# sihan-shao/QuantizationAwareTHzDOE

Measured on AMD Instinct MI355X. Metric: complex-field propagations/sec (N×N) + achieved HBM GB/s at 1/2/4/8 GPU, higher is better.
Workload: dtype complex64 (fp32)

## Files before the change

include/thzdoe.h:

```cpp
#ifndef THZDOE_H_
#define THZDOE_H_

#include <stddef.h>

#ifdef __cplusplus
extern "C" {
#endif

#define THZ_OK 0
#define THZ_E_ARG 1
#define THZ_E_UNSUPPORTED 2
#define THZ_E_WORKSPACE 3
#define THZ_E_HIP 4

#define THZ_BANDLIMIT_NONE 0
#define THZ_BANDLIMIT_EXACT 1
#define THZ_BANDLIMIT_APPROX 2

#define THZ_MAX_WAVELENGTHS 64
#define THZ_MAX_Z 256

typedef void* thz_stream_t;

#define THZ_ABI_VERSION 9

const char* thz_version(void);
const char* thz_last_error(void);
int thz_abi_version(void);

typedef struct thz_asm_desc {
  int B, C, H, W;
  int pad_h, pad_w;
  int unpad;
  int bandlimit;
  int Z;
  int adjoint;
  int z_chunk;
  float dx, dy;
  const float* wavelengths;
  const float* z;
  const struct thz_aperture_desc* window_mask;
  const float* z_dev;
} thz_asm_desc;

int thz_asm_workspace_size(const thz_asm_desc* d, size_t* bytes);
int thz_asm_forward(const thz_asm_desc* d, const void* in, void* out, void* workspace, size_t workspace_bytes,
                    thz_stream_t stream);
int thz_asm_slice_workspace_size(const thz_asm_desc* d, size_t* bytes);
int thz_asm_slice_forward(const thz_asm_desc* d, int row, const void* in, void* out ,
                          void* workspace, size_t workspace_bytes, thz_stream_t stream);
int thz_asm_slice_adjoint_workspace_size(const thz_asm_desc* d, size_t* bytes);
int thz_asm_slice_adjoint(const thz_asm_desc* d, int row, const void* grad_out ,
                          void* grad_in , void* workspace, size_t workspace_bytes,
                          thz_stream_t stream);
int thz_asm_band(const thz_asm_desc* d, int* ncols, int* z_chunk);
int thz_asm_transfer_function(const thz_asm_desc* d, void* out, thz_stream_t stream);

typedef struct thz_czt_desc {
  int B, C, H, W;
  int outH, outW;
  float dx, dy;
  float odx, ody;
  float z;
  const float* wavelengths;
  int adjoint;
} thz_czt_desc;

int thz_czt_workspace_size(const thz_czt_desc* d, size_t* bytes);
int thz_czt_forward(const thz_czt_desc* d, const void* in, void* out, void* workspace, size_t workspace_bytes,
                    thz_stream_t stream);

typedef struct thz_czt_slice_desc {
  int B, C, H, W;
  int outH, outW;
  float dx, dy, odx, ody;
  int Z;
  const float* z;
  const float* wavelengths;
  int row;
} thz_czt_slice_desc;

int thz_czt_slice_workspace_size(const thz_czt_slice_desc* d, size_t* bytes);
int thz_czt_slice_forward(const thz_czt_slice_desc* d, const void* in ,
                          void* out , void* workspace, size_t workspace_bytes,
                          thz_stream_t stream);
int thz_czt_slice_adjoint_workspace_size(const thz_czt_slice_desc* d, size_t* bytes);
int thz_czt_slice_adjoint(const thz_czt_slice_desc* d, const void* grad_out ,
                          void* grad_in , void* workspace, size_t workspace_bytes,
                          thz_stream_t stream);

typedef struct thz_rsc_desc {
  int B, C, H, W;
  int vectorial;
  float dx, dy;
  float z;
  const float* wavelengths;
  int adjoint;
} thz_rsc_desc;

int thz_rsc_workspace_size(const thz_rsc_desc* d, size_t* bytes);
int thz_rsc_forward(const thz_rsc_desc* d, const void* in, void* out, void* workspace, size_t workspace_bytes,
                    thz_stream_t stream);

typedef struct thz_rsc_slice_desc {
  int B, C, H, W;
  int vectorial;
  float dx, dy;
  int Z;
// ... 202 lines not shown
```

quantizationawarethzdoe_amd/_lib.py:

```python
from __future__ import annotations

import ctypes
import os
import threading

_HERE = os.path.dirname(os.path.abspath(__file__))
LIB_PATH = os.environ.get("THZDOE_LIB", os.path.join(_HERE, "libthzdoe.so"))

THZ_OK = 0
THZ_E_ARG = 1
THZ_E_UNSUPPORTED = 2
THZ_E_WORKSPACE = 3
THZ_E_HIP = 4
THZ_MAX_WAVELENGTHS = 64
THZ_MAX_Z = 256
THZ_ABI_VERSION = 9

BANDLIMIT = {None: 0, False: 0, "none": 0, "exact": 1, "approx": 2}

EXPORTED = [
    "thz_version", "thz_last_error", "thz_abi_version",
    "thz_asm_workspace_size", "thz_asm_forward", "thz_asm_band", "thz_asm_forward_modulated",
    "thz_asm_forward_loss", "thz_asm_adjoint_loss", "thz_asm_transfer_function", "thz_rs_kernel",
    "thz_asm_slice_workspace_size", "thz_asm_slice_forward",
    "thz_asm_slice_adjoint_workspace_size", "thz_asm_slice_adjoint",
    "thz_czt_workspace_size", "thz_czt_forward",
    "thz_czt_slice_workspace_size", "thz_czt_slice_forward",
    "thz_czt_slice_adjoint_workspace_size", "thz_czt_slice_adjoint",
    "thz_rsc_workspace_size", "thz_rsc_forward",
    "thz_rsc_slice_workspace_size", "thz_rsc_slice_forward",
    "thz_rsc_slice_adjoint_workspace_size", "thz_rsc_slice_adjoint",
    "thz_doe_modulate_forward", "thz_doe_modulate_backward", "thz_quant_forward", "thz_quant_backward",
    "thz_doe_quant_backward", "thz_radial_quant_backward",
    "thz_radial_forward", "thz_radial_backward",
    "thz_gaussian_beam", "thz_thin_lens", "thz_aperture",
    "thz_intensity_mse_workspace_size", "thz_intensity_mse_forward", "thz_intensity_mse_backward",
    "thz_resample_forward", "thz_resample_backward",
    "thz_fft_rows",
    "thz_asm64_workspace_size", "thz_asm64_forward", "thz_czt64_workspace_size", "thz_czt64_forward",
    "thz_rsc64_workspace_size", "thz_rsc64_forward", "thz_fft64_rows",
    "thz_step_fetch", "thz_adam_step",
    "thz_timing_enable", "thz_timing_reset", "thz_timing_read",
]


class ThzError(RuntimeError):

    def __init__(self, code, msg):
        super().__init__(f"libthzdoe error {code}: {msg}")
        self.code = code


class AsmDesc(ctypes.Structure):
    _fields_ = [
        ("B", ctypes.c_int), ("C", ctypes.c_int), ("H", ctypes.c_int), ("W", ctypes.c_int),
        ("pad_h", ctypes.c_int), ("pad_w", ctypes.c_int),
        ("unpad", ctypes.c_int), ("bandlimit", ctypes.c_int), ("Z", ctypes.c_int),
        ("adjoint", ctypes.c_int), ("z_chunk", ctypes.c_int),
        ("dx", ctypes.c_float), ("dy", ctypes.c_float),
        ("wavelengths", ctypes.POINTER(ctypes.c_float)), ("z", ctypes.POINTER(ctypes.c_float)),
        ("window_mask", ctypes.c_void_p),
        ("z_dev", ctypes.c_void_p),
    ]


class CztDesc(ctypes.Structure):
    _fields_ = [
        ("B", ctypes.c_int), ("C", ctypes.c_int), ("H", ctypes.c_int), ("W", ctypes.c_int),
        ("outH", ctypes.c_int), ("outW", ctypes.c_int),
        ("dx", ctypes.c_float), ("dy", ctypes.c_float), ("odx", ctypes.c_float), ("ody", ctypes.c_float),
        ("z", ctypes.c_float), ("wavelengths", ctypes.POINTER(ctypes.c_float)), ("adjoint", ctypes.c_int),
    ]


class CztSliceDesc(ctypes.Structure):
# ... 151 lines not shown
    lib.thz_asm_forward_loss.argtypes = [ctypes.POINTER(AsmDesc), ctypes.POINTER(DoeDesc), c_void_p, c_void_p,
                                         c_void_p, c_void_p, ctypes.POINTER(LossDesc), c_void_p, c_void_p, c_void_p,
                                         c_void_p, c_void_p, c_size_t, c_void_p]
    lib.thz_asm_adjoint_loss.argtypes = [ctypes.POINTER(AsmDesc), ctypes.POINTER(LossDesc), c_void_p, c_void_p,
                                         c_void_p, c_void_p, c_void_p, c_void_p, c_void_p, c_size_t, c_void_p]
    lib.thz_fft_rows.argtypes = [c_void_p, c_void_p, c_int, c_int, c_int, c_void_p]
    lib.thz_rsc_workspace_size.argtypes = [ctypes.POINTER(RscDesc), ctypes.POINTER(c_size_t)]
    lib.thz_rsc_forward.argtypes = [ctypes.POINTER(RscDesc), c_void_p, c_void_p, c_void_p, c_size_t, c_void_p]
    lib.thz_rsc_slice_workspace_size.argtypes = [ctypes.POINTER(RscSliceDesc), ctypes.POINTER(c_size_t)]
    lib.thz_rsc_slice_forward.argtypes = [ctypes.POINTER(RscSliceDesc), c_void_p, c_void_p, c_void_p, c_size_t,
                                          c_void_p]
    lib.thz_rsc_slice_adjoint_workspace_size.argtypes = [ctypes.POINTER(RscSliceDesc), ctypes.POINTER(c_size_t)]
    lib.thz_rsc_slice_adjoint.argtypes = [ctypes.POINTER(RscSliceDesc), c_void_p, c_void_p, c_void_p, c_size_t,
                                          c_void_p]
    lib.thz_doe_modulate_forward.argtypes = [ctypes.POINTER(DoeDesc), c_void_p, c_void_p, c_void_p, c_void_p,
                                             c_void_p, c_void_p]
    lib.thz_doe_modulate_backward.argtypes = [ctypes.POINTER(DoeDesc), c_void_p, c_void_p, c_void_p, c_void_p,
                                              c_void_p, c_void_p, c_void_p]
    lib.thz_quant_forward.argtypes = [ctypes.POINTER(QuantDesc), c_void_p, c_void_p, c_void_p, c_void_p, c_void_p]
    lib.thz_quant_backward.argtypes = [ctypes.POINTER(QuantDesc), c_void_p, c_void_p, c_void_p, c_void_p, c_void_p]
    lib.thz_doe_quant_backward.argtypes = [ctypes.POINTER(DoeDesc), ctypes.POINTER(QuantDesc), c_void_p, c_void_p,
                                           c_void_p, c_void_p, c_void_p, c_void_p, c_void_p, c_void_p, c_void_p]
    lib.thz_radial_quant_backward.argtypes = [ctypes.POINTER(QuantDesc), c_void_p, c_int, c_int, c_int, c_void_p,
                                              c_void_p, c_void_p, c_void_p]
    lib.thz_radial_forward.argtypes = [c_void_p, c_int, c_int, c_int, c_void_p, c_void_p]
    lib.thz_radial_backward.argtypes = [c_void_p, c_int, c_int, c_int, c_void_p, c_void_p]
    lib.thz_czt_workspace_size.argtypes = [ctypes.POINTER(CztDesc), ctypes.POINTER(c_size_t)]
    lib.thz_czt_forward.argtypes = [ctypes.POINTER(CztDesc), c_void_p, c_void_p, c_void_p, c_size_t, c_void_p]
    lib.thz_czt_slice_workspace_size.argtypes = [ctypes.POINTER(CztSliceDesc), ctypes.POINTER(c_size_t)]
    lib.thz_czt_slice_forward.argtypes = [ctypes.POINTER(CztSliceDesc), c_void_p, c_void_p, c_void_p, c_size_t,
                                          c_void_p]
    lib.thz_czt_slice_adjoint_workspace_size.argtypes = [ctypes.POINTER(CztSliceDesc), ctypes.POINTER(c_size_t)]
    lib.thz_czt_slice_adjoint.argtypes = [ctypes.POINTER(CztSliceDesc), c_void_p, c_void_p, c_void_p, c_size_t,
                                          c_void_p]
    lib.thz_gaussian_beam.argtypes = [ctypes.POINTER(GaussDesc), c_void_p, c_void_p]
    lib.thz_thin_lens.argtypes = [ctypes.POINTER(LensDesc), c_void_p, c_void_p, c_void_p]
    lib.thz_aperture.argtypes = [ctypes.POINTER(ApertureDesc), c_void_p, c_void_p, c_void_p]
    lib.thz_asm_transfer_function.argtypes = [ctypes.POINTER(AsmDesc), c_void_p, c_void_p]
    lib.thz_rs_kernel.argtypes = [c_void_p, c_void_p, c_int, ctypes.c_float, c_void_p, c_int, c_void_p, c_void_p]
    lib.thz_intensity_mse_workspace_size.argtypes = [ctypes.POINTER(LossDesc)]
    lib.thz_intensity_mse_forward.argtypes = [ctypes.POINTER(LossDesc), c_void_p, c_void_p, c_void_p, c_void_p,
                                              c_void_p]
    lib.thz_intensity_mse_backward.argtypes = [ctypes.POINTER(LossDesc), c_void_p, c_void_p, c_void_p, c_void_p,
                                               c_void_p, c_void_p]
    lib.thz_resample_forward.argtypes = [ctypes.POINTER(ResampleDesc), c_void_p, c_void_p, c_void_p]
    lib.thz_resample_backward.argtypes = [ctypes.POINTER(ResampleDesc), c_void_p, c_void_p, c_void_p]
    for tag, desc in (("asm64", AsmDesc64), ("czt64", CztDesc64), ("rsc64", RscDesc64)):
        getattr(lib, f"thz_{tag}_workspace_size").argtypes = [ctypes.POINTER(desc), ctypes.POINTER(c_size_t)]
        getattr(lib, f"thz_{tag}_forward").argtypes = [ctypes.POINTER(desc), c_void_p, c_void_p, c_void_p, c_size_t,
                                                       c_void_p]
    lib.thz_fft64_rows.argtypes = [c_void_p, c_void_p, c_int, c_int, c_int, c_void_p]
    lib.thz_step_fetch.argtypes = [c_void_p, c_int, c_int, c_void_p, c_void_p, c_void_p]
    lib.thz_adam_step.argtypes = [ctypes.POINTER(AdamDesc), ctypes.POINTER(AdamParam), c_void_p]
    lib.thz_timing_enable.argtypes = [c_int]
    lib.thz_timing_reset.argtypes = []
    lib.thz_timing_read.argtypes = [ctypes.c_char_p, ctypes.POINTER(ctypes.c_double), ctypes.POINTER(ctypes.c_long)]
    for name in EXPORTED[2:]:
        getattr(lib, name).restype = c_int
    lib.thz_intensity_mse_workspace_size.restype = c_size_t


def lib():
    global _lib
    if _lib is None:
        with _lock:
            if _lib is None:
                if not os.path.exists(LIB_PATH):
                    raise ThzError(-1, f"{LIB_PATH} not built: run __graft_entry__.build() "
                                       "(make -C quantizationawarethzdoe_amd/csrc)")
                h = ctypes.CDLL(LIB_PATH)
                _declare(h)
                abi = h.thz_abi_version()
                if abi != THZ_ABI_VERSION:
                    raise ThzError(-1, f"{LIB_PATH} has ABI {abi}, these bindings describe ABI {THZ_ABI_VERSION}: "
                                       "rebuild the library (make -C quantizationawarethzdoe_amd/csrc)")
                _lib = h
    return _lib


def check(code):
    if code != THZ_OK:
        raise ThzError(code, lib().thz_last_error().decode())


def version():
    return lib().thz_version().decode()


def timing_enable(on=True):
    check(lib().thz_timing_enable(int(bool(on))))


def timing_reset():
    check(lib().thz_timing_reset())


def timing_read(kernel):
    ms, n = ctypes.c_double(0), ctypes.c_long(0)
    check(lib().thz_timing_read(kernel.encode(), ctypes.byref(ms), ctypes.byref(n)))
    return ms.value, n.value


def double_array(values):
    return (ctypes.c_double * max(1, len(values)))(*[float(v) for v in values])


def float_array(values):
    arr = (ctypes.c_float * max(1, len(values)))(*[float(v) for v in values])
    return arr
```

quantizationawarethzdoe_amd/csrc/thz_asm.hip:

```cpp
#include <algorithm>
#include <map>
#include <mutex>
#include <cmath>
#include <cstdlib>
#include <tuple>
#include <vector>

#include "thz_common.hpp"
#include "thz_dev.hpp"
#include "thz_wfft.hpp"


namespace thz {

__device__ __forceinline__ void st_stream(float2* p, float2 v) {
  typedef float f32x2 __attribute__((ext_vector_type(2)));
  __builtin_nontemporal_store(f32x2{v.x, v.y}, reinterpret_cast<f32x2*>(p));
}

constexpr float TWO_PI_F = 6.283185307179586f;

struct AsmArgs {
  int BC, C;
  int Ph, Pw;
  int in_r0, in_c0, Hin, Win;
  int out_r0, out_c0, Hout, Wout;
  int ncols, J;
  int ncb;
  int ncbu;
  int nz, zoff;
  int kfull, kparts;
  int bl, adjoint;
  int zsum, zacc;
  int zrec;
  float dx, dy, scale;
  const float2* tft;
  int vec;
  float zr;
  float* sqt;
  int* mzt;
  const float* mod_h;
  const float* mod_u;
  float* mod_hfull;
  int mod_hs, mod_ws;
  float mod_tol, mod_eps, mod_tand;
  const unsigned* mod_rng;
  unsigned mod_rng_stream;
  LossSink ls;
  const float2* lg_field;
  const float* lg_gloss;
  const float* lg_target;
  const float* lg_stats;
  int lg_tB, lg_tC;
// ... 818 lines not shown
    const int c0 = tid + a.J;
    const float2* base = src + blk_u(c0, r, a.Hout);
    const long cstride = u_rows(a.Hout);
    static_assert(NB0 == PN / 16, "radix-16 first stage");
    const bool mid0 = __all(c0 + 4 * NB0 >= a.ncols && c0 + 11 * NB0 - PN < 0);
    auto ld = [&](int, int q, int) {
      if (q >= 4 && q < 12 && mid0) return make_float2(0.f, 0.f);
      const int delta = q * NB0 >= PN / 2 ? q * NB0 - PN : q * NB0;
      if ((unsigned)(c0 + delta) >= (unsigned)a.ncols) return make_float2(0.f, 0.f);
      return base[(long)delta * cstride];
    };
    auto sv = [&](int, int, int j, float2 v) {
      const int w = j - (MID ? PN / 4 : a.out_c0);
      if ((unsigned)w < (unsigned)(MID ? PN / 2 : a.Wout)) put(w, v);
    };
    fft_pow2_run<true, PN, TT, FFT_ROWS>(lds, twl, tid, ld, sv, tw_hook);
  } else {
    for (int j = tid; j < a.Pw; j += nt) {
      const int c = band_col(j, a.Pw, a.J, a.ncols);
      lds[padx(j)] = c >= 0 ? src[blk_u(c, r, a.Hout)] : make_float2(0.f, 0.f);
    }
    __syncthreads();
    fft_lds<true>(lds, pw, tid, nt);
    for (int w = tid; w < a.Wout; w += nt) put(w, lds[padx(a.out_c0 + w)]);
  }
  if constexpr (LOSS) loss_store_part(acc, a.ls, lb, lc * a.Hout + r);
}

template <int PN>
__global__ void __launch_bounds__(1024) THZ_ROW_ATTR asm_rows_inv(const float2* __restrict__ U, float2* __restrict__ out,
                                                    FftPlan pw, AsmArgs a) {
  rows_inv_body<PN, false>(U, out, pw, a);
}

template <int PN>
__global__ void __launch_bounds__(1024) THZ_ROW_ATTR asm_rows_inv_mid(const float2* __restrict__ U,
                                                                      float2* __restrict__ out, FftPlan pw, AsmArgs a) {
  rows_inv_body<PN, false, true>(U, out, pw, a);
}

template <int PN>
__global__ void __launch_bounds__(1024) THZ_ROW_ATTR asm_rows_inv_loss_mid(const float2* __restrict__ U,
                                                                           float2* __restrict__ out, FftPlan pw,
                                                                           AsmArgs a) {
  rows_inv_body<PN, true, true>(U, out, pw, a);
}

template <int PN>
__global__ void __launch_bounds__(1024) THZ_ROW_ATTR asm_rows_inv_loss(const float2* __restrict__ U,
                                                                       float2* __restrict__ out, FftPlan pw, AsmArgs a) {
  rows_inv_body<PN, true>(U, out, pw, a);
}

constexpr int SLICE_ZC = 64;

template <int PN>
__global__ void __launch_bounds__(1024) asm_cols_slice(const float2* __restrict__ T, float2* __restrict__ V,
                                                      FftPlan ph, AsmArgs a, int R) {
  extern __shared__ float2 lds[];
  using S = Pow2Sched<PN>;
  constexpr int TT = Geo<PN>::T;
  static_assert(S::radix(S::NST - 1, true) == 16 && PN / 16 / TT == 1, "one radix-16 butterfly per thread");
  int id, z_lo, z_hi;
  k2_task(a, id, z_lo, z_hi);
  const int bc = id / a.ncols, c = id - bc * a.ncols;
  const int nt = blockDim.x, nz = z_hi - z_lo;
  const float2* col = T + (size_t)bc * a.ncb * CB * a.Hin + blk(c, 0, a.Hin);
  const float lam = a.lam[bc % a.C];
  const float Ky = kfreq(c - a.J, a.Pw, a.dy);
  const int tid = threadIdx.x;
  float2 sp[16];
  const TwLds twl = load_tw_lds<PN>(lds + lds_floats2(PN), ph.tw, threadIdx.x, blockDim.x);
  auto ld0 = [&](int, int, int idx) {
    const int s = idx - a.in_r0;
    return (s >= 0 && s < a.Hin) ? col[(size_t)s * CB] : make_float2(0.f, 0.f);
  };
  auto sv0 = [&](int, int r, int, float2 v) { sp[r] = v; };
  fft_pow2_io<false, PN, TT, true, false, false>(lds, twl, tid, ld0, sv0);
#pragma unroll
  for (int r = 0; r < 16; ++r) sp[r] = cmul(cscale(sp[r], a.scale), slice_row_phase<PN>(tid, r, R));
  const auto [mz, zok, zl] = col_lds<PN>(lds);
  const float kl = TWO_PI_F / lam;
  const float kl2 = tf_mul(kl, kl);
  const float Ky2 = tf_mul(Ky, Ky);
  for (int zz = tid; zz < nz; zz += nt) {
    const float zq = zval(a, a.zoff + z_lo + zz);
    zl[zz] = zq;
    mz[zz] = tf_band_bound<PN>(a, a.Ph, tf_scalars(a, lam, zq), Ky);
    zok[zz] = recurrence_votes([&](int q) { return zval(a, a.zoff + z_lo + q); }, zz, nz, kl);
  }
  float sq[16];
#pragma unroll
  for (int r = 0; r < 16; ++r) sq[r] = col_sq<PN>(tid + r * (PN / 16), a, kl2, Ky2);
  __syncthreads();
  bool rec, rev;
  recurrence_order<PN>(mz, zok, nz, a.zrec, rec, rev);
  const int lane = threadIdx.x & 63;
  float2* part = lds;
  const int wave = threadIdx.x >> 6, nw = nt >> 6;
  float2 dstep[8];
  float dz = 0.f, zprev = 0.f;
  int Mprev = -2;
  const int zfirst = rev ? nz - 1 : 0, zstep = rev ? -1 : 1;
  if (rec) {
    const float z0 = zl[zfirst];
    dz = zl[zfirst + zstep] - z0;
// ... 716 lines not shown
static bool on_listed(SizeList<Ns...>, int n, F&& f) {
  return ((n == Ns ? (f(Size<Ns>{}), true) : false) || ...);
}
template <class F, int... Ns>
static void for_each_size(SizeList<Ns...>, F&& f) {
  (f(Size<Ns>{}), ...);
}
template <class F>
static bool on_pow2_only(int n, F&& f) {
  return on_listed(Pow2Sizes{}, n, f);
}
template <class F>
static void on_pow2(int n, F&& f) {
  if (!on_listed(Pow2Sizes{}, n, f)) f(Size<0>{});
}
template <class F>
static void on_rows(int n, F&& f) {
  if (!on_listed(SizeList<Mx300::N, Mx500::N>{}, n, f)) on_pow2(n, f);
}
template <class F>
static void on_mx(int n, F&& f) {
  if (n == Mx300::N) f(Mx300{});
  else f(Mx500{});
}

static int pow2_kind(int n) { return on_pow2_only(n, [](auto) {}) ? n : 0; }
static int threads_for(int n) { return pow2_kind(n) ? n / pow2_v(n) : fft_threads(n); }
static int rows_threads(int n) { return is_mx(n) ? mx_threads(n) : threads_for(n); }

static size_t k2_lds_bytes(int Ph) { return fft_lds_bytes(Ph) + 12 * THZ_MAX_Z; }
static size_t k2_zsum_lds_bytes(int Ph) { return fft_lds_bytes(Ph) + 4 * THZ_MAX_Z; }
static size_t k2_mx_lds_bytes(int Ph) { return lds_floats2(Ph) * sizeof(float2) + 4 * THZ_MAX_Z; }

static int ensure_lds_attr() {
  static std::once_flag once;
  static hipError_t err = hipSuccess;
  std::call_once(once, [] {
    const int mx = (int)k2_lds_bytes(FFT_MAX_N);
    std::vector<const void*> ks;
    auto planes = [&](auto N) {
      constexpr int PN = N();
      ks.insert(ks.end(), {(const void*)asm_rows_fwd<PN>, (const void*)asm_cols<PN>, (const void*)asm_cols_zsum<PN>,
                           (const void*)asm_rows_inv<PN>, (const void*)asm_rows_inv_loss<PN>,
                           (const void*)asm_rows_slice<PN>, (const void*)fft_rows_kernel<PN>,
                           (const void*)rsc_k_rows<PN>, (const void*)rsc_k_cols<PN>,
                           (const void*)rsc_slice_rows<PN>, (const void*)rsc_slice_line<PN>,
                           (const void*)rsc_slice_line_adj<PN>, (const void*)rsc_slice_rows_adj<PN, false>});
      if constexpr (PN == 0 || rss_acc_compiled(PN))
        ks.insert(ks.end(), {(const void*)rsc_slice_acc<PN, 1>, (const void*)rsc_slice_acc_adj<PN, 1>,
                             (const void*)rsc_slice_rows_adj<PN, true>});
      if constexpr (rss_acc_compiled(PN))
        ks.insert(ks.end(), {(const void*)rsc_slice_acc<PN, 2>, (const void*)rsc_slice_acc<PN, 3>,
                             (const void*)rsc_slice_acc_adj<PN, 2>, (const void*)rsc_slice_acc_adj<PN, 3>});
      if constexpr (PN == 8192) ks.push_back((const void*)asm_rows_inv_mid<PN>);
    };
    for_each_size(Pow2Sizes{}, planes);
    planes(Size<0>{});
    for_each_size(Pow2Sizes{}, [&](auto N) {
      ks.insert(ks.end(), {(const void*)asm_cols_slice<N()>, (const void*)asm_cols_slice_adj<N()>});
    });
    for (const void* k : ks) {
      hipError_t e = hipFuncSetAttribute(k, hipFuncAttributeMaxDynamicSharedMemorySize, mx);
      if (e != hipSuccess) err = e;
    }
  });
  if (err != hipSuccess) return fail(THZ_E_HIP, "hipFuncSetAttribute(MaxDynamicSharedMemorySize): %s",
                                     hipGetErrorString(err));
  return THZ_OK;
}

static size_t align256(size_t x) { return (x + 255) & ~(size_t)255; }

static bool mx_mid(int Ph, const AsmArgs& a) {
  return Ph == Mx300::N && !a.tft && a.in_r0 == Mx300::N / 3 && a.Hin == Mx300::N / 3 && a.out_r0 == Mx300::N / 3 &&
         a.Hout == Mx300::N / 3;
}
static bool k3_mid(int Pw, const AsmArgs& a) {
  return (Pw == 8192 && a.out_c0 == Pw / 4 && a.Wout == Pw / 2) ||
         (Pw == Mx300::N && a.out_c0 == Pw / 3 && a.Wout == Pw / 3);
}
static bool k1_mid(int Pw, const AsmArgs& a) { return Pw == Mx300::N && a.in_c0 == Pw / 3 && a.Win == Pw / 3; }

using PassKernel = void (*)(const float2*, float2*, FftPlan, AsmArgs);

static PassKernel cols_kernel(int Ph) {
  PassKernel k = nullptr;
  if (is_mx(Ph)) on_mx(Ph, [&](auto P) { k = asm_cols_mx<decltype(P)>; });
  else on_pow2(Ph, [&](auto N) { k = asm_cols<N()>; });
  return k;
}

static int k2_resident(int Ph, int threads, size_t lds) {
  static std::mutex mu;
  static std::map<std::tuple<int, int, int, size_t>, int> cache;
  int dev = 0;
  if (hipGetDevice(&dev) != hipSuccess) return 0;
  std::lock_guard<std::mutex> lk(mu);
  auto key = std::make_tuple(dev, Ph, threads, lds);
  auto it = cache.find(key);
  if (it != cache.end()) return it->second;
  int per_cu = 0, cus = 0;
  if (hipOccupancyMaxActiveBlocksPerMultiprocessor(&per_cu, (const void*)cols_kernel(Ph), threads, lds) != hipSuccess ||
      hipDeviceGetAttribute(&cus, hipDeviceAttributeMultiprocessorCount, dev) != hipSuccess)
    per_cu = cus = 0;
  const int r = per_cu * cus;
  cache[key] = r;
  return r;
// ... 63 lines not shown
  FftPlan pw, ph;
  AsmArgs a;
  hipStream_t s;
  int Z;
  char* ws[3];
};

static int launch_k1(const AsmPlan& p, const AsmArgs& a, int planes, const void* in, float2* T) {
  const int Pw = p.g.Pw;
  PassKernel k = nullptr;
  if (k1_mid(Pw, a)) k = asm_rows_fwd<Mx300::N, true>;
  else on_rows(Pw, [&](auto N) { k = asm_rows_fwd<N()>; });
  KernelTimer kt("asm_rows_fwd", p.s);
  hipLaunchKernelGGL(k, dim3(planes * a.BC * a.Hin + a.tab_blocks), dim3(rows_threads(Pw)), fft_lds_bytes_io(Pw), p.s,
                     (const float2*)in, T, p.pw, a);
  THZ_LAUNCH_CHECK();
  kt.stop();
  return THZ_OK;
}

static int launch_cols(const AsmPlan& p, AsmArgs& a, bool tables, const float2* T, float2* U) {
  const AsmGeom& g = p.g;
  const bool mx = is_mx(g.Ph);
  const int th = mx ? mx_threads(g.Ph) : threads_for(g.Ph);
  const size_t lds = mx ? k2_mx_lds_bytes(g.Ph) : a.zsum ? k2_zsum_lds_bytes(g.Ph) : k2_lds_bytes(g.Ph);
  PassKernel k = nullptr;
  if (a.zsum) {
    if (mx) on_mx(g.Ph, [&](auto P) { k = asm_cols_mx_zsum<decltype(P)>; });
    else on_pow2(g.Ph, [&](auto N) { k = asm_cols_zsum<N()>; });
  } else {
    k = mx_mid(g.Ph, a) ? asm_cols_mx_mid<Mx300> : cols_kernel(g.Ph);
  }
  KernelTimer kt("asm_cols", p.s);
  if (tables) {
    on_mx(g.Ph, [&](auto P) {
      hipLaunchKernelGGL(asm_tf_tables<decltype(P)::N>, dim3(g.C * g.ncols), dim3(MX_T), 0, p.s, a, a.zoff == 0);
    });
    THZ_LAUNCH_CHECK();
  }
  int ntask = g.ncols * g.BC;
  if (a.zsum) {
    a.kfull = ntask;
    a.kparts = 1;
  } else {
    ntask = k2_tasks(g, &a, th, lds);
    if (!mx) a.zrec = !plane_recurrence_disabled();
  }
  hipLaunchKernelGGL(k, dim3(ntask), dim3(th), lds, p.s, T, U, p.ph, a);
  THZ_LAUNCH_CHECK();
  kt.stop();
  return THZ_OK;
}

static int launch_k3(const AsmPlan& p, const AsmArgs& a, const float2* U, void* out) {
  const int Pw = p.g.Pw;
  const bool loss = a.ls.stats != nullptr, mid = k3_mid(Pw, a);
  PassKernel k = nullptr;
  if (mid && Pw == Mx300::N) k = loss ? asm_rows_inv_loss_mid<Mx300::N> : asm_rows_inv_mid<Mx300::N>;
  else if (mid && !loss) k = asm_rows_inv_mid<8192>;
  else if (loss) on_rows(Pw, [&](auto N) { k = asm_rows_inv_loss<N()>; });
  else on_rows(Pw, [&](auto N) { k = asm_rows_inv<N()>; });
  KernelTimer kt("asm_rows_inv", p.s);
  hipLaunchKernelGGL(k, dim3(a.nz * a.BC * a.Hout), dim3(rows_threads(Pw)), fft_lds_bytes_io(Pw), p.s, U, (float2*)out,
                     p.pw, a);
  THZ_LAUNCH_CHECK();
  int e;
  if (loss && (e = launch_loss_finish(a.ls, p.s))) return e;
  kt.stop();
  return THZ_OK;
}

static int launch_cols_slice(const AsmPlan& p, AsmArgs& a, bool adjoint, const float2* src, float2* dst, int R) {
  const AsmGeom& g = p.g;
  const int th = threads_for(g.Ph);
  const size_t lds = k2_lds_bytes(g.Ph);
  void (*k)(const float2*, float2*, FftPlan, AsmArgs, int) = nullptr;
  const bool served = on_pow2_only(g.Ph, [&](auto N) {
    if (adjoint) k = asm_cols_slice_adj<N()>;
    else k = asm_cols_slice<N()>;
  });
  if (!served) return fail(THZ_E_UNSUPPORTED, "z-x slice: no column pass for padded height %d", g.Ph);
  a.zrec = !plane_recurrence_disabled();
  KernelTimer kt(adjoint ? "asm_cols_slice_adj" : "asm_cols_slice", p.s);
  const int ntask = adjoint ? g.ncols * g.BC : k2_tasks(g, &a, th, lds);
  hipLaunchKernelGGL(k, dim3(ntask), dim3(th), lds, p.s, src, dst, p.ph, a, R);
  THZ_LAUNCH_CHECK();
  kt.stop();
  return THZ_OK;
}

static int launch_rows_slice(const AsmPlan& p, const AsmArgs& a, const float2* V, void* out) {
  const int Pw = p.g.Pw;
  PassKernel k = nullptr;
  on_pow2(Pw, [&](auto N) { k = asm_rows_slice<N()>; });
  KernelTimer kt("asm_rows_slice", p.s);
  hipLaunchKernelGGL(k, dim3(a.nz * a.BC), dim3(threads_for(Pw)), fft_lds_bytes_io(Pw), p.s, V, (float2*)out, p.pw, a);
  THZ_LAUNCH_CHECK();
  kt.stop();
  return THZ_OK;
}

static int run_adjoint_sum(const AsmPlan& p, AsmArgs a, const void* in, void* out) {
  float2 *T = (float2*)p.ws[0], *U = (float2*)p.ws[1];
  int e;
  a.zsum = 1;
  a.tab_blocks = 0;
  for (int z0 = 0; z0 < p.Z; z0 += p.g.zc) {
    a.zoff = z0;
    a.nz = std::min(p.g.zc, p.Z - z0);
    a.zacc = z0 > 0;
    if ((e = launch_k1(p, a, a.nz, in, T))) return e;
    if ((e = launch_cols(p, a, a.sqt != nullptr, T, U))) return e;
  }
  a.zoff = 0;
  a.nz = 1;
  return launch_k3(p, a, U, out);
}
// ... 81 lines not shown
      return fail(THZ_E_ARG, "z-x slice%s: row %d outside [0, %d)", pipe == Pipe::Slice ? "" : " adjoint", row, rows);
  }
  if (!data_ok) return fail(THZ_E_ARG, "null data pointer");
  const WsLayout lay = ws_layout(pipe, g, d->Z);
  if ((e = check_workspace(workspace, bytes, lay.total()))) return e;
  if ((e = device_plans(g, &p->pw, &p->ph))) return e;
  char* w = (char*)workspace;
  for (int i = 0; i < 3; ++i) {
    p->ws[i] = lay.part[i] ? w : nullptr;
    w += lay.part[i];
  }
  p->a = asm_args_base(d, g);
  p->s = (hipStream_t)stream;
  p->Z = d->Z;
  return THZ_OK;
}

static int asm_workspace_size(const thz_asm_desc* d, Pipe pipe, size_t* bytes) {
  int e = validate_pipe(d, pipe);
  if (e) return e;
  if (!bytes) return fail(THZ_E_ARG, "null bytes");
  AsmGeom g;
  geometry(d, &g);
  *bytes = ws_layout(pipe, g, d->Z).total();
  return THZ_OK;
}

}

using namespace thz;

extern "C" int thz_asm_slice_workspace_size(const thz_asm_desc* d, size_t* bytes) {
  return asm_workspace_size(d, Pipe::Slice, bytes);
}

extern "C" int thz_asm_slice_forward(const thz_asm_desc* d, int row, const void* in, void* out, void* workspace,
                                     size_t workspace_bytes, thz_stream_t stream) {
  AsmPlan p;
  int e = asm_plan(d, Pipe::Slice, row, in && out, workspace, workspace_bytes, stream, &p);
  if (e) return e;
  return run_slice(p, row + p.a.out_r0, in, out);
}

extern "C" int thz_asm_slice_adjoint_workspace_size(const thz_asm_desc* d, size_t* bytes) {
  return asm_workspace_size(d, Pipe::SliceAdjoint, bytes);
}

extern "C" int thz_asm_slice_adjoint(const thz_asm_desc* d, int row, const void* grad_out, void* grad_in,
                                     void* workspace, size_t workspace_bytes, thz_stream_t stream) {
  AsmPlan p;
  int e = asm_plan(d, Pipe::SliceAdjoint, row, grad_out && grad_in, workspace, workspace_bytes, stream, &p);
  if (e) return e;
  return run_slice_adjoint(p, row + p.a.in_r0, grad_out, grad_in);
}

extern "C" int thz_asm_band(const thz_asm_desc* d, int* ncols, int* z_chunk) {
  int e = validate(d);
  if (e) return e;
  AsmGeom g;
  geometry(d, &g);
  if (ncols) *ncols = g.ncols;
  if (z_chunk) *z_chunk = g.zc;
  return THZ_OK;
}

extern "C" int thz_asm_workspace_size(const thz_asm_desc* d, size_t* bytes) {
  return asm_workspace_size(d, Pipe::Planes, bytes);
}

namespace thz {
struct AsmFused {
  struct {
    const thz_doe_desc* desc;
    const float *height, *noise;
    float* height_full;
  } mod{};
  const LossSink* loss = nullptr;
  struct {
    const thz_loss_desc* desc;
    const float2* field;
    const float *target, *stats, *gloss;
  } grad{};
};

static int check_doe_desc(const thz_asm_desc* d, const thz_doe_desc* m) {
  if (m->B != d->B || m->C != d->C || m->H != d->H || m->W != d->W)
    return fail(THZ_E_ARG, "DOE field %dx%dx%dx%d does not match the ASM input %dx%dx%dx%d", m->B, m->C, m->H, m->W,
                d->B, d->C, d->H, d->W);
  if (m->hs < 1 || m->ws < 1) return fail(THZ_E_ARG, "bad height-map size %dx%d", m->hs, m->ws);
  return THZ_OK;
}

static int check_loss_desc(const thz_asm_desc* d, const thz_loss_desc* l) {
  const int Ho = d->unpad ? d->H : d->H + 2 * d->pad_h, Wo = d->unpad ? d->W : d->W + 2 * d->pad_w;
  if (l->B != d->Z * d->B || l->C != d->C || l->H != Ho || l->W != Wo)
    return fail(THZ_E_ARG, "loss field %dx%dx%dx%d does not match the ASM output %dx%dx%dx%d", l->B, l->C, l->H, l->W,
                d->B, d->C, Ho, Wo);
  if (!(l->tB == 1 || l->tB == l->B) || !(l->tC == 1 || l->tC == l->C))
    return fail(THZ_E_ARG, "target %dx%d does not broadcast over %dx%d", l->tB, l->tC, l->B, l->C);
  return THZ_OK;
}

static int asm_forward_impl(const thz_asm_desc* d, const void* in, void* out, void* workspace, size_t workspace_bytes,
                            thz_stream_t stream, const AsmFused& f) {
  AsmPlan p;
  int e = asm_plan(d, Pipe::Planes, 0, (in || f.grad.field) && out, workspace, workspace_bytes, stream, &p);
// ... 460 lines not shown
```

quantizationawarethzdoe_amd/csrc/thz_common.hpp:

```cpp
#pragma once
#include <hip/hip_runtime.h>

#include <cstdarg>
#include <cstdio>
#include <string>

#include "../../include/thzdoe.h"
#include "thz_fft.hpp"

namespace thz {

void set_error(const char* fmt, ...);
int fail(int code, const char* fmt, ...);

#define THZ_HIP_CHECK(expr)                                                                  \
  do {                                                                                       \
    hipError_t _e = (expr);                                                                  \
    if (_e != hipSuccess)                                                                    \
      return ::thz::fail(THZ_E_HIP, "%s failed: %s (%s:%d)", #expr, hipGetErrorString(_e),   \
                         __FILE__, __LINE__);                                                \
  } while (0)

#define THZ_LAUNCH_CHECK() THZ_HIP_CHECK(hipGetLastError())

constexpr int FFT_MAX_N = 16384;

int get_plan(int n, FftPlan* out);

struct KernelTimer {
  const char* name;
  hipStream_t stream;
  hipEvent_t start = nullptr;
  KernelTimer(const char* n, hipStream_t s);
  void stop();
};

int fft_rows_strided(const void* in, void* out, int rows, int n, size_t stride, int inverse, hipStream_t s);

inline int fft_threads(int n) {
  int t = (n + FFT_MAXV - 1) / FFT_MAXV;
  t = (t + 63) / 64 * 64;
  if (t < 64) t = 64;
  return t;
}
inline size_t fft_lds_bytes(int n) { return (size_t)(lds_floats2(n) + tw_lds_count(n)) * sizeof(float2); }
inline size_t fft_lds_bytes_io(int n) {
  const bool pow2 = n >= 1024 && n <= 16384 && (n & (n - 1)) == 0;
  if (pow2) return (size_t)(lds_split_f2(n) + tw_lds_count(n)) * sizeof(float2);
  return fft_lds_bytes(n);
}

}
```

quantizationawarethzdoe_amd/csrc/thz_fft.hpp:

```cpp
#pragma once
#include <hip/hip_runtime.h>

#include <type_traits>
#include <utility>

namespace thz {

constexpr int FFT_MAX_STAGES = 24;
__host__ __device__ constexpr int row_waves_per_eu(int n) { return n >= 8192 ? 8 : 1; }
#define THZ_ROW_ATTR __attribute__((amdgpu_waves_per_eu(row_waves_per_eu(PN))))
constexpr int FFT_MAXV = 16;
__host__ __device__ constexpr int pow2_v(int) { return 16; }
constexpr int pow2_log(int v) { return v <= 1 ? 0 : 1 + pow2_log(v >> 1); }

struct FftPlan {
  int n;
  int nst;
  int radix[FFT_MAX_STAGES];
  const float2* tw;
};

__device__ __forceinline__ int padx(int a) { return a + (a >> 4); }
__host__ __device__ constexpr int lds_floats2(int n) { return n + (n >> 4) + 1; }

// ... 665 lines not shown
      __syncthreads();
#pragma unroll
      for (int m = 0; m < MB; ++m) {
        const int i = tid + m * T;
        const int k = i & (L - 1);
        const int i0 = m * T, k0 = i0 & (L - 1), j0 = (i0 - k0) * R + k0;
        float* dst = lds + split_lay<L>((i - k) * R + k);
#pragma unroll
        for (int r = 0; r < R; ++r)
          dst[split_lay<L>(j0 + r * L) - split_lay<L>(j0)] = part ? v[m][r].y : v[m][r].x;
      }
      __syncthreads();
      if constexpr (PAIR) {
        constexpr int LP = N / 32;
        const float* src = lds + split_lay<L>(pair_i(tid) + ((tid >> 5) & 1) * LP);
#pragma unroll
        for (int s = 0; s < 16; ++s) {
          const float x = src[split_lay<L>(2 * s * LP) - split_lay<L>(0)];
          if (part) nx[0][s].y = x;
          else nx[0][s].x = x;
        }
      } else {
#pragma unroll
        for (int m = 0; m < MB2; ++m) {
          const float* src = lds + split_lay<L>(tid + m * T);
#pragma unroll
          for (int r = 0; r < R2; ++r) {
            const float x = src[split_lay<L>(m * T + r * NB2) - split_lay<L>(m * T)];
            if (part) nx[m][r].y = x;
            else nx[m][r].x = x;
          }
        }
      }
    }
    if constexpr (PAIR) {
      stage_r32_pair_last<INV, N>(tw, tid, nx[0], sv);
    } else {
      auto in2 = [&](int m, int r, int) { return nx[m][r]; };
      fft_pow2_split_io<INV, N, T, MODE, S + 1, L * R>(lds, tw, tid, in2, sv);
    }
  }
  }
}

template <int N>
__device__ __forceinline__ float2* tw_slot(float2* lds) {
  return lds + lds_split_f2(N);
}
template <bool INV, int N, int T, int MODE, class Tw, class Ld, class Sv, class Hook = NoHook>
__device__ __forceinline__ void fft_pow2_run(float2* lds, const Tw& tw, int tid, Ld& ld, Sv& sv, Hook hook = Hook{}) {
  fft_pow2_split_io<INV, N, T, MODE>(reinterpret_cast<float*>(lds), tw, tid, ld, sv, hook);
}

template <bool INV, int N, int T, class Tw>
__device__ __forceinline__ void fft_pow2(float2* lds, const Tw& tw, int tid) {
  NoIO io;
  fft_pow2_io<INV, N, T, false, true, true>(lds, tw, tid, io, io);
}

template <bool INV, int N, int T, int L, int R, bool FIRST, bool LAST, int MW, class Ld, class Sv>
__device__ __forceinline__ void mx_stage(float2* lds, const float2 (&w1)[MW], const float2* __restrict__ tw, int tid,
                                         Ld& ld, Sv& sv) {
  constexpr int NB = N / R;
  constexpr int MB = (NB + T - 1) / T;
  static_assert(MB <= MW, "mixed plan: twiddle registers");
  float2 v[MB][R];
#pragma unroll
  for (int m = 0; m < MB; ++m) {
    const int i = tid + m * T;
    if (NB % T == 0 || i < NB) {
#pragma unroll
      for (int r = 0; r < R; ++r) {
        if constexpr (FIRST) v[m][r] = ld(m, r, i + r * NB);
        else v[m][r] = lds[i + r * NB];
      }
      if constexpr (L > 1) {
        const float2 w = w1[m];
        float2 wr = w;
#pragma unroll
        for (int r = 1; r < R; ++r) {
          v[m][r] = cmul_tw<INV>(v[m][r], wr);
          if (r + 1 < R) wr = cmul(wr, w);
        }
      }
      dftR<R, INV>(v[m]);
    }
  }
  if constexpr (LAST) {
    static_assert(L * R == N, "mixed plan: radices must multiply to N");
#pragma unroll
    for (int m = 0; m < MB; ++m) {
      const int i = tid + m * T;
      if (NB % T == 0 || i < NB) {
#pragma unroll
        for (int r = 0; r < R; ++r) sv(m, r, i + r * NB, v[m][r]);
      }
    }
  } else {
    __syncthreads();
#pragma unroll
    for (int m = 0; m < MB; ++m) {
      const int i = tid + m * T;
      if (NB % T == 0 || i < NB) {
        const int k = i % L;
        const int j = (i - k) * R + k;
#pragma unroll
// ... 87 lines not shown
```

Measured before the change: 8106.

## Process two output rows per block in the inverse row FFT pass

Adds a paired-row variant of the inverse row FFT kernel in which each block loads adjacent rows 2i and 2i+1 with a single float4 read from the shared U tile and runs both FFTs together, sharing twiddles and synchronisation. The grid is halved and LDS doubles to hold two line images. By default it is enabled only for the mid-band 8192 case, and a runtime mode switch can force it on or off. The aim is to cut load instructions, twiddle work and barriers per row, at the cost of higher register and LDS pressure, which lowers occupancy.

```diff
diff --git a/include/thzdoe.h b/include/thzdoe.h
--- a/include/thzdoe.h
+++ b/include/thzdoe.h
@@ -54,6 +54,7 @@
                           void* grad_in , void* workspace, size_t workspace_bytes,
                           thz_stream_t stream);
 int thz_asm_band(const thz_asm_desc* d, int* ncols, int* z_chunk);
+int thz_asm_row_pairs(int mode);
 int thz_asm_transfer_function(const thz_asm_desc* d, void* out, thz_stream_t stream);
 
 typedef struct thz_czt_desc {
diff --git a/quantizationawarethzdoe_amd/_lib.py b/quantizationawarethzdoe_amd/_lib.py
--- a/quantizationawarethzdoe_amd/_lib.py
+++ b/quantizationawarethzdoe_amd/_lib.py
@@ -20,7 +20,7 @@
 
 EXPORTED = [
     "thz_version", "thz_last_error", "thz_abi_version",
-    "thz_asm_workspace_size", "thz_asm_forward", "thz_asm_band", "thz_asm_forward_modulated",
+    "thz_asm_workspace_size", "thz_asm_forward", "thz_asm_band", "thz_asm_row_pairs", "thz_asm_forward_modulated",
     "thz_asm_forward_loss", "thz_asm_adjoint_loss", "thz_asm_transfer_function", "thz_rs_kernel",
     "thz_asm_slice_workspace_size", "thz_asm_slice_forward",
     "thz_asm_slice_adjoint_workspace_size", "thz_asm_slice_adjoint",
@@ -278,6 +278,7 @@
     lib.thz_fft64_rows.argtypes = [c_void_p, c_void_p, c_int, c_int, c_int, c_void_p]
     lib.thz_step_fetch.argtypes = [c_void_p, c_int, c_int, c_void_p, c_void_p, c_void_p]
     lib.thz_adam_step.argtypes = [ctypes.POINTER(AdamDesc), ctypes.POINTER(AdamParam), c_void_p]
+    lib.thz_asm_row_pairs.argtypes = [c_int]
     lib.thz_timing_enable.argtypes = [c_int]
     lib.thz_timing_reset.argtypes = []
     lib.thz_timing_read.argtypes = [ctypes.c_char_p, ctypes.POINTER(ctypes.c_double), ctypes.POINTER(ctypes.c_long)]
@@ -317,6 +318,10 @@
     check(lib().thz_timing_enable(int(bool(on))))
 
 
+def asm_row_pairs(mode=-1):
+    check(lib().thz_asm_row_pairs(int(mode)))
+
+
 def timing_reset():
     check(lib().thz_timing_reset())
 
diff --git a/quantizationawarethzdoe_amd/csrc/thz_asm.hip b/quantizationawarethzdoe_amd/csrc/thz_asm.hip
--- a/quantizationawarethzdoe_amd/csrc/thz_asm.hip
+++ b/quantizationawarethzdoe_amd/csrc/thz_asm.hip
@@ -1,4 +1,5 @@
 #include <algorithm>
+#include <atomic>
 #include <map>
 #include <mutex>
 #include <cmath>
@@ -923,6 +924,55 @@
   rows_inv_body<PN, true>(U, out, pw, a);
 }
 
+template <int PN, bool MID>
+__device__ __forceinline__ void rows_inv_pair_body(const float2* __restrict__ U, float2* __restrict__ out, FftPlan pw,
+                                                   const AsmArgs& a) {
+  static_assert(PN >= 1024 && !is_mx(PN), "power-of-two sizes");
+  static_assert(URT % 2 == 0, "rows 2i and 2i + 1 share a U tile");
+  extern __shared__ float2 lds[];
+  constexpr int TT = Geo<PN>::T;
+  const int hp = (a.Hout + 1) >> 1;
+  const int pr = xcd_rows(blockIdx.x, gridDim.x);
+  const int plane = pr / hp, r = 2 * (pr - plane * hp);
+  const bool two = r + 1 < a.Hout;
+  const int tid = threadIdx.x;
+  __builtin_assume(tid >= 0 && tid < TT);
+  const float2* src = U + (size_t)plane * a.ncbu * CBU * u_rows(a.Hout);
+  float2* dst0 = out + ((size_t)(a.zoff * a.BC + plane) * a.Hout + r) * a.Wout;
+  float2* dst1 = dst0 + a.Wout;
+  const auto twf = tw_fetch<PN, TT>(pw.tw, tid);
+  const TwLds twl = tw_lds_at<PN>(tw_slot2<PN>(lds));
+  auto tw_hook = [&]() { tw_store<PN, TT>(tw_slot2<PN>(lds), twf, tid); };
+  constexpr int NB0 = PN / pow2_v(PN);
+  static_assert(NB0 % CBU == 0, "band offsets must be whole U blocks");
+  static_assert(Geo<PN>::T == NB0 && NB0 == PN / 16, "radix-16 first stage, one butterfly per thread");
+  const int c0 = tid + a.J;
+  const float2* base = src + blk_u(c0, r, a.Hout);
+  const long cstride = u_rows(a.Hout);
+  const bool mid0 = __all(c0 + 4 * NB0 >= a.ncols && c0 + 11 * NB0 - PN < 0);
+  auto ld = [&](int, int q, int, float2& x0, float2& x1) {
+    x0 = x1 = make_float2(0.f, 0.f);
+    if (q >= 4 && q < 12 && mid0) return;
+    const int delta = q * NB0 >= PN / 2 ? q * NB0 - PN : q * NB0;
+    if ((unsigned)(c0 + delta) >= (unsigned)a.ncols) return;
+    const float4 x = *reinterpret_cast<const float4*>(base + (long)delta * cstride);
+    x0 = make_float2(x.x, x.y);
+    if (two) x1 = make_float2(x.z, x.w);
+  };
+  auto sv = [&](int line, int, int, int j, float2 v) {
+    const int w = j - (MID ? PN / 4 : a.out_c0);
+    if ((unsigned)w < (unsigned)(MID ? PN / 2 : a.Wout) && (line == 0 || two)) st_stream((line ? dst1 : dst0) + w, v);
+  };
+  fft_pow2_run2<true, PN, TT, FFT_ROWS>(lds, twl, tid, ld, sv, tw_hook);
+}
+
+constexpr int pair_waves_per_eu(int n) { return n == 4096 ? 3 : 4; }
+template <int PN, bool MID>
+__global__ void __launch_bounds__(Geo<PN>::T) __attribute__((amdgpu_waves_per_eu(pair_waves_per_eu(PN))))
+asm_rows_inv_pair(const float2* __restrict__ U, float2* __restrict__ out, FftPlan pw, AsmArgs a) {
+  rows_inv_pair_body<PN, MID>(U, out, pw, a);
+}
+
 constexpr int SLICE_ZC = 64;
 
 template <int PN>
@@ -1745,7 +1795,9 @@
       if constexpr (rss_acc_compiled(PN))
         ks.insert(ks.end(), {(const void*)rsc_slice_acc<PN, 2>, (const void*)rsc_slice_acc<PN, 3>,
                              (const void*)rsc_slice_acc_adj<PN, 2>, (const void*)rsc_slice_acc_adj<PN, 3>});
-      if constexpr (PN == 8192) ks.push_back((const void*)asm_rows_inv_mid<PN>);
+      if constexpr (PN == 8192)
+        ks.insert(ks.end(), {(const void*)asm_rows_inv_mid<PN>, (const void*)asm_rows_inv_pair<PN, true>});
+      if constexpr (PN > 0) ks.push_back((const void*)asm_rows_inv_pair<PN, false>);
     };
     for_each_size(Pow2Sizes{}, planes);
     planes(Size<0>{});
@@ -1915,17 +1967,28 @@
   return THZ_OK;
 }
 
+static std::atomic<int> g_row_pairs{-1};
+
+static bool k3_pairs(int Pw, bool loss, bool mid) {
+  if (loss || !pow2_kind(Pw)) return false;
+  const int mode = g_row_pairs.load(std::memory_order_relaxed);
+  return mode < 0 ? mid && Pw == 8192 : mode > 0;
+}
+
 static int launch_k3(const AsmPlan& p, const AsmArgs& a, const float2* U, void* out) {
   const int Pw = p.g.Pw;
-  const bool loss = a.ls.stats != nullptr, mid = k3_mid(Pw, a);
+  const bool loss = a.ls.stats != nullptr, mid = k3_mid(Pw, a), pairs = k3_pairs(Pw, loss, mid);
   PassKernel k = nullptr;
   if (mid && Pw == Mx300::N) k = loss ? asm_rows_inv_loss_mid<Mx300::N> : asm_rows_inv_mid<Mx300::N>;
+  else if (pairs && mid) k = asm_rows_inv_pair<8192, true>;
+  else if (pairs) on_pow2_only(Pw, [&](auto N) { k = asm_rows_inv_pair<N(), false>; });
   else if (mid && !loss) k = asm_rows_inv_mid<8192>;
   else if (loss) on_rows(Pw, [&](auto N) { k = asm_rows_inv_loss<N()>; });
   else on_rows(Pw, [&](auto N) { k = asm_rows_inv<N()>; });
   KernelTimer kt("asm_rows_inv", p.s);
-  hipLaunchKernelGGL(k, dim3(a.nz * a.BC * a.Hout), dim3(rows_threads(Pw)), fft_lds_bytes_io(Pw), p.s, U, (float2*)out,
-                     p.pw, a);
+  const int rows = pairs ? (a.Hout + 1) / 2 : a.Hout;
+  hipLaunchKernelGGL(k, dim3(a.nz * a.BC * rows), dim3(rows_threads(Pw)), fft_lds_bytes_io(Pw, pairs ? 2 : 1), p.s, U,
+                     (float2*)out, p.pw, a);
   THZ_LAUNCH_CHECK();
   int e;
   if (loss && (e = launch_loss_finish(a.ls, p.s))) return e;
@@ -2113,6 +2176,12 @@
   int e = asm_plan(d, Pipe::SliceAdjoint, row, grad_out && grad_in, workspace, workspace_bytes, stream, &p);
   if (e) return e;
   return run_slice_adjoint(p, row + p.a.in_r0, grad_out, grad_in);
+}
+
+extern "C" int thz_asm_row_pairs(int mode) {
+  if (mode < -1 || mode > 1) return fail(THZ_E_ARG, "thz_asm_row_pairs: mode %d (-1, 0 or 1)", mode);
+  g_row_pairs.store(mode, std::memory_order_relaxed);
+  return THZ_OK;
 }
 
 extern "C" int thz_asm_band(const thz_asm_desc* d, int* ncols, int* z_chunk) {
diff --git a/quantizationawarethzdoe_amd/csrc/thz_common.hpp b/quantizationawarethzdoe_amd/csrc/thz_common.hpp
--- a/quantizationawarethzdoe_amd/csrc/thz_common.hpp
+++ b/quantizationawarethzdoe_amd/csrc/thz_common.hpp
@@ -44,9 +44,9 @@
   return t;
 }
 inline size_t fft_lds_bytes(int n) { return (size_t)(lds_floats2(n) + tw_lds_count(n)) * sizeof(float2); }
-inline size_t fft_lds_bytes_io(int n) {
+inline size_t fft_lds_bytes_io(int n, int lines = 1) {
   const bool pow2 = n >= 1024 && n <= 16384 && (n & (n - 1)) == 0;
-  if (pow2) return (size_t)(lds_split_f2(n) + tw_lds_count(n)) * sizeof(float2);
+  if (pow2) return (size_t)(lines * lds_split_f2(n) + tw_lds_count(n)) * sizeof(float2);
   return fft_lds_bytes(n);
 }
 
diff --git a/quantizationawarethzdoe_amd/csrc/thz_fft.hpp b/quantizationawarethzdoe_amd/csrc/thz_fft.hpp
--- a/quantizationawarethzdoe_amd/csrc/thz_fft.hpp
+++ b/quantizationawarethzdoe_amd/csrc/thz_fft.hpp
@@ -741,6 +741,120 @@
   fft_pow2_split_io<INV, N, T, MODE>(reinterpret_cast<float*>(lds), tw, tid, ld, sv, hook);
 }
 
+template <int R, bool INV, int N, int L, int T, class Tw, class In>
+__device__ __forceinline__ void stage_core2(const Tw& tw, int tid, In& in, float2 (&v)[2][N / R / T][R]) {
+  constexpr int NB = N / R;
+  constexpr int MB = NB / T;
+  static_assert(MB * T == NB, "pow2 plan must tile exactly");
+  constexpr int TWS = N / (L * R);
+#pragma unroll
+  for (int m = 0; m < MB; ++m) {
+    const int i = tid + m * T;
+#pragma unroll
+    for (int r = 0; r < R; ++r) in(m, r, i + r * NB, v[0][m][r], v[1][m][r]);
+    if constexpr (L > 1) {
+      if constexpr (L * R == 256 && std::is_same<Tw, TwLds>::value) {
+        static_assert(L == 16, "the L R = 256 stage of a radix-16 schedule");
+        const int k = i & (L - 1);
+#pragma unroll
+        for (int r = 1; r < R; ++r) {
+          const float2 w = tw.t256[16 * r + k];
+          v[0][m][r] = cmul_tw<INV>(v[0][m][r], w);
+          v[1][m][r] = cmul_tw<INV>(v[1][m][r], w);
+        }
+      } else {
+        float2 w[R];
+        twiddle_powers<R>(tw, (i & (L - 1)) * TWS, w);
+#pragma unroll
+        for (int r = 1; r < R; ++r) {
+          v[0][m][r] = cmul_tw<INV>(v[0][m][r], w[r]);
+          v[1][m][r] = cmul_tw<INV>(v[1][m][r], w[r]);
+        }
+      }
+    }
+    dftR<R, INV>(v[0][m]);
+    dftR<R, INV>(v[1][m]);
+  }
+}
+
+template <bool INV, int N, int T, int MODE, int LS, int S = 0, int L = 1, class Tw, class In, class Sv,
+          class Hook = NoHook>
+__device__ __forceinline__ void fft_pow2_split2_io(float* lds, const Tw& tw, int tid, In& in, Sv& sv,
+                                                   Hook hook = Hook{}) {
+  using P = Pow2Sched<N>;
+  constexpr int R = P::radix(S, MODE);
+  static_assert(R <= 16, "two-line form: no lane-pair stage");
+  static_assert(LS >= 2 * lds_split_f2(N), "line 1's image starts behind line 0's");
+  constexpr int MB = N / R / T;
+  float2 v[2][MB][R];
+  stage_core2<R, INV, N, L, T>(tw, tid, in, v);
+  if constexpr (S == 0) hook();
+  if constexpr (S == P::nst(MODE) - 1) {
+#pragma unroll
+    for (int m = 0; m < MB; ++m) {
+      const int i = tid + m * T;
+#pragma unroll
+      for (int r = 0; r < R; ++r) {
+        sv(0, m, r, i + r * L, v[0][m][r]);
+        sv(1, m, r, i + r * L, v[1][m][r]);
+      }
+    }
+  } else {
+    constexpr int R2 = P::radix(S + 1, MODE);
+    static_assert(R2 <= 16, "two-line form: no lane-pair stage");
+    constexpr int NB2 = N / R2;
+    constexpr int MB2 = NB2 / T;
+    static_assert(split_lay<L>(N - 1) < 2 * lds_split_f2(N), "split layout exceeds the LDS image");
+    float2 nx[2][MB2][R2];
+#pragma unroll
+    for (int part = 0; part < 2; ++part) {
+      __syncthreads();
+#pragma unroll
+      for (int m = 0; m < MB; ++m) {
+        const int i = tid + m * T;
+        const int k = i & (L - 1);
+        const int i0 = m * T, k0 = i0 & (L - 1), j0 = (i0 - k0) * R + k0;
+        float* dst = lds + split_lay<L>((i - k) * R + k);
+#pragma unroll
+        for (int line = 0; line < 2; ++line)
+#pragma unroll
+          for (int r = 0; r < R; ++r)
+            dst[line * LS + split_lay<L>(j0 + r * L) - split_lay<L>(j0)] = part ? v[line][m][r].y : v[line][m][r].x;
+      }
+      __syncthreads();
+#pragma unroll
+      for (int m = 0; m < MB2; ++m) {
+        const float* src = lds + split_lay<L>(tid + m * T);
+#pragma unroll
+        for (int line = 0; line < 2; ++line)
+#pragma unroll
+          for (int r = 0; r < R2; ++r) {
+            const float x = src[line * LS + split_lay<L>(m * T + r * NB2) - split_lay<L>(m * T)];
+            if (part) nx[line][m][r].y = x;
+            else nx[line][m][r].x = x;
+          }
+      }
+    }
+    auto in2 = [&](int m, int r, int, float2& x0, float2& x1) {
+      x0 = nx[0][m][r];
+      x1 = nx[1][m][r];
+    };
+    fft_pow2_split2_io<INV, N, T, MODE, LS, S + 1, L * R>(lds, tw, tid, in2, sv);
+  }
+}
+template <int N>
+__host__ __device__ constexpr int pair_line_floats() {
+  return 2 * lds_split_f2(N);
+}
+template <int N>
+__device__ __forceinline__ float2* tw_slot2(float2* lds) {
+  return lds + 2 * lds_split_f2(N);
+}
+template <bool INV, int N, int T, int MODE, class Tw, class Ld, class Sv, class Hook = NoHook>
+__device__ __forceinline__ void fft_pow2_run2(float2* lds, const Tw& tw, int tid, Ld& ld, Sv& sv, Hook hook = Hook{}) {
+  fft_pow2_split2_io<INV, N, T, MODE, pair_line_floats<N>()>(reinterpret_cast<float*>(lds), tw, tid, ld, sv, hook);
+}
+
 template <bool INV, int N, int T, class Tw>
 __device__ __forceinline__ void fft_pow2(float2* lds, const Tw& tw, int tid) {
   NoIO io;
```

Result: faster. 8251, median of 6 (+1.8%).
